# wathiede/pbrt

Hardware: AMD Instinct MI355X
Metric: Msamples/sec (rays/sec) at 1/2/4/8 GPUs; PSNR vs CPU reference (higher is better)
Workload: dtype f32

## Files before the change

pbrt_amd/csrc/kernel_walk.hpp:

```cpp
#pragma once
#include <cstdio>
#include <cstdlib>
#include <vector>

#include "device_types.h"
#include "kernel_math.hpp"

namespace pbrt_hip {
namespace {

constexpr uint32_t kDone = 0xffffffffu;

typedef __attribute__((address_space(3))) uint32_t lds_u32;
__device__ __forceinline__ uint32_t lds_addr(const uint32_t *p) { return (uint32_t)(uintptr_t)(const lds_u32 *)p; }
__device__ __forceinline__ void lds_store(uint32_t a, uint32_t v) { *(lds_u32 *)(uintptr_t)a = v; }
__device__ __forceinline__ uint32_t lds_load(uint32_t a) { return *(const lds_u32 *)(uintptr_t)a; }
constexpr uint32_t kRowBytes = 256u;
__device__ __forceinline__ uint32_t lane_here() { uint32_t l = threadIdx.x & 63u; asm volatile("" : "+v"(l)); return l; }
__device__ __forceinline__ uint32_t lds_row(uint32_t a, const uint32_t *stk) { return (a - lds_addr(stk - (threadIdx.x & 63u))) / kRowBytes; }

struct Trav {
  V3 o, d;
  float tmax;
  uint32_t cur;
  uint32_t sp;
  uint32_t any;
  HitRec h;
};

struct TravTuning {
  uint32_t min_walkers;
  uint32_t min_parked;
};

#ifndef PBRT_PRIO_FETCH
#define PBRT_PRIO_FETCH 3
#endif
#ifndef PBRT_PRIO_ARITH
#define PBRT_PRIO_ARITH 0
#endif
#ifndef PBRT_PRIO_SERVICE
#define PBRT_PRIO_SERVICE 1
#endif
__device__ __forceinline__ void wave_prio(int p) {
#ifndef PBRT_NO_PRIO
  switch (p) {
    case 0: __builtin_amdgcn_s_setprio(0); break;
    case 1: __builtin_amdgcn_s_setprio(1); break;
    case 2: __builtin_amdgcn_s_setprio(2); break;
    default: __builtin_amdgcn_s_setprio(3); break;
  }
#endif
}

__device__ __forceinline__ bool box_test(float lx, float ly, float lz, float hx, float hy, float hz, V3 o, V3 inv,
                                         bool negx, bool negy, bool negz, float tfar, float &tn) {
  const float nx = ((negx ? hx : lx) - o.x) * inv.x, fx = ((negx ? lx : hx) - o.x) * inv.x;
  const float ny = ((negy ? hy : ly) - o.y) * inv.y, fy = ((negy ? ly : hy) - o.y) * inv.y;
  const float nz = ((negz ? hz : lz) - o.z) * inv.z, fz = ((negz ? lz : hz) - o.z) * inv.z;
  tn = fmaxf(fmaxf(nx, ny), fmaxf(nz, kRayTMin));
  const float tf = fminf(fminf(fx, fy), fminf(fz, tfar));
  return tn <= tf * kBoxPad;
}

template <bool EXACT, uint32_t OVFR>
__device__ __forceinline__ uint32_t trav_pop(Trav &T, uint32_t *stk, float *stkt, uint32_t *ovf, unsigned long long &cn) {
  if (EXACT) {
    while (T.sp != 0u) {
      T.sp--;
      const uint32_t ref = stk[T.sp * 64u];
      const float tn = stkt[T.sp * 64u];
      cn++;
      if (tn <= fminf(T.h.t, T.tmax) * kBoxPad) return ref;
    }
    return kDone;
  }
  T.sp -= kRowBytes;
  if (OVFR == 0u) return lds_load(T.sp);
  const uint32_t e = lds_row(T.sp, stk);
  return e < OVFR - 1u ? lds_load(T.sp) : ovf[(e - (OVFR - 1u)) * 64u + lane_here()];
}
template <uint32_t OVFR>
__device__ __forceinline__ void trav_push(Trav &T, uint32_t *stk, uint32_t *ovf, uint32_t ref) {
  if (OVFR == 0u) {
    lds_store(T.sp, ref);
  } else {
    const uint32_t e = lds_row(T.sp, stk);
    if (e < OVFR - 1u) lds_store(T.sp, ref);
    else ovf[(e - (OVFR - 1u)) * 64u + lane_here()] = ref;
  }
  T.sp += kRowBytes;
}

__device__ __forceinline__ void trav_enter(Trav &T, uint32_t ref) { T.cur = ref; }
__device__ __forceinline__ bool trav_parked(const Trav &T) { return T.cur != kDone && (T.cur & kLeafRef) != 0u; }
__device__ __forceinline__ uint32_t trav_leaf_cnt(const Trav &T) { return trav_parked(T) ? (T.cur >> 24) & 0x7fu : 0u; }

#include "experiments.inc"
template <bool EXACT>
__device__ __forceinline__ void trav_begin(const DevScene &S, Trav &T, uint32_t *stk, V3 o, V3 d, float tmax, bool any,
                                           unsigned long long &cn) {
  T.o = o;
  T.d = d;
  T.tmax = tmax;
  T.sp = 0;
  if (!EXACT) {
    lds_store(lds_addr(stk), kDone);
    T.sp = lds_addr(stk) + kRowBytes;
  }
  T.any = any ? 1u : 0u;
  T.h.t = kInf;
  T.h.prim = kNoPrim;
  T.h.slot = kNoPrim;
  T.h.b1 = 0.f;
  T.h.b2 = 0.f;
  T.cur = kDone;
  if (S.n_nodes) {
    if (EXACT) cn++;
    if (!EXACT && o.x >= S.root_lo[0] && o.x <= S.root_hi[0] && o.y >= S.root_lo[1] && o.y <= S.root_hi[1] && o.z >= S.root_lo[2] &&
        o.z <= S.root_hi[2]) {
      trav_enter(T, !(S.root_ref & kLeafRef) ? 0u : S.root_ref);
      return;
    }
    const V3 inv = {1.0f / d.x, 1.0f / d.y, 1.0f / d.z};
    float tn;
    if (box_test(S.root_lo[0], S.root_lo[1], S.root_lo[2], S.root_hi[0], S.root_hi[1], S.root_hi[2], o, inv,
                 inv.x < 0.f, inv.y < 0.f, inv.z < 0.f, tmax, tn))
      trav_enter(T, (!EXACT && !(S.root_ref & kLeafRef)) ? 0u : S.root_ref);
  }
}

__device__ __forceinline__ V3 walk_inv(const V3 d, const V3 inv1, const float inv_parallel) {
  return V3{d.x == 0.f ? copysignf(inv_parallel, inv1.x) : inv1.x, d.y == 0.f ? copysignf(inv_parallel, inv1.y) : inv1.y,
            d.z == 0.f ? copysignf(inv_parallel, inv1.z) : inv1.z};
}

template <bool SCALAR_FMA>
__device__ __forceinline__ void quad_step(const uint4 W0, const uint4 W1, const uint4 W2, const V3 o, const V3 inv, const bool negx,
                                          const bool negy, const bool negz, const float tfar, float (&key)[4], bool (&hit)[4]) {
  const float gx = (o.x - __uint_as_float(W0.x)) * inv.x, gy = (o.y - __uint_as_float(W0.y)) * inv.y;
  const float gz = (o.z - __uint_as_float(W0.z)) * inv.z;
  constexpr float kMargin = 0x1.8p-22f;
  const float gxn = __builtin_fmaf(fabsf(gx), kMargin, gx), gxf = __builtin_fmaf(-fabsf(gx), kMargin, gx);
  const float gyn = __builtin_fmaf(fabsf(gy), kMargin, gy), gyf = __builtin_fmaf(-fabsf(gy), kMargin, gy);
  const float gzn = __builtin_fmaf(fabsf(gz), kMargin, gz), gzf = __builtin_fmaf(-fabsf(gz), kMargin, gz);
  const float cix = __uint_as_float(W0.w) * inv.x, ciy = __uint_as_float(W2.z) * inv.y, ciz = __uint_as_float(W2.w) * inv.z;
  const uint32_t bnx = negx ? W1.w : W1.x, bfx = negx ? W1.x : W1.w;
  const uint32_t bny = negy ? W2.x : W1.y, bfy = negy ? W1.y : W2.x;
  const uint32_t bnz = negz ? W2.y : W1.z, bfz = negz ? W1.z : W2.y;
  const f32x2 gxx = {gxn, gxf}, gyy = {gyn, gyf}, gzz = {gzn, gzf}, cxx = {cix, cix}, cyy = {ciy, ciy}, czz = {ciz, ciz};
#pragma unroll
  for (int k = 0; k < 4; k++) {
    const float qxn = (float)((bnx >> (8 * k)) & 0xffu), qxf = (float)((bfx >> (8 * k)) & 0xffu);
    const float qyn = (float)((bny >> (8 * k)) & 0xffu), qyf = (float)((bfy >> (8 * k)) & 0xffu);
    const float qzn = (float)((bnz >> (8 * k)) & 0xffu), qzf = (float)((bfz >> (8 * k)) & 0xffu);
    f32x2 tx, ty, tz;
    if (SCALAR_FMA) {
      tx = f32x2{__builtin_fmaf(qxn, cix, -gxn), __builtin_fmaf(qxf, cix, -gxf)};
      ty = f32x2{__builtin_fmaf(qyn, ciy, -gyn), __builtin_fmaf(qyf, ciy, -gyf)};
      tz = f32x2{__builtin_fmaf(qzn, ciz, -gzn), __builtin_fmaf(qzf, ciz, -gzf)};
    } else {
      tx = __builtin_elementwise_fma(f32x2{qxn, qxf}, cxx, -gxx);
      ty = __builtin_elementwise_fma(f32x2{qyn, qyf}, cyy, -gyy);
      tz = __builtin_elementwise_fma(f32x2{qzn, qzf}, czz, -gzz);
    }
    const float tn = fmaxf(fmaxf(tx.x, ty.x), fmaxf(tz.x, kRayTMin));
    const float tf = fminf(fminf(tx.y, ty.y), fminf(tz.y, tfar));
    hit[k] = tn <= tf * kBoxPad;
    key[k] = tn;
  }
}

template <bool EXACT, bool COUNT, uint32_t OVFR, int STEPS = PBRT_STEPS_PER_CHECK, bool SPH = false>
__device__ __forceinline__ void trav_run(const DevScene &S, Trav &T, uint32_t *stk, float *stkt, uint32_t *ovf,
                                         const bool alive, const TravTuning tune, unsigned long long &cn,
                                         unsigned long long &ct) {
  const V3 o = T.o, d = T.d;
  const V3 inv1 = {1.0f / d.x, 1.0f / d.y, 1.0f / d.z};
  const bool negx = inv1.x < 0.f, negy = inv1.y < 0.f, negz = inv1.z < 0.f;
  const uint32_t negbits = (negx ? 1u : 0u) | (negy ? 2u : 0u) | (negz ? 4u : 0u);
#ifdef PBRT_INV_INF
  const V3 inv = inv1;
#else
  const V3 inv = EXACT ? inv1 : walk_inv(d, inv1, S.inv_parallel);
#endif
  const char *nodes = reinterpret_cast<const char *>(S.nodes);
  const char *quads = reinterpret_cast<const char *>(S.quads);
  const char *tris = reinterpret_cast<const char *>(S.tris);
  for (;;) {
    const bool walking = T.cur != kDone;
    const unsigned long long mwalk = __ballot(walking);
    if (mwalk == 0ull) break;
    if ((uint32_t)__popcll(mwalk) * 64u < tune.min_walkers * (uint32_t)__popcll(__ballot(alive)) && __ballot(!walking && alive) != 0ull) break;

    if (EXACT && walking && !trav_parked(T)) {
      const uint32_t off = T.cur * 64u;
      const uint4 q0 = *reinterpret_cast<const uint4 *>(nodes + off);
      const uint4 q1 = *reinterpret_cast<const uint4 *>(nodes + off + 16u);
      const uint4 q2 = *reinterpret_cast<const uint4 *>(nodes + off + 32u);
      const uint4 q3 = *reinterpret_cast<const uint4 *>(nodes + off + 48u);
      const float tfar = fminf(T.h.t, T.tmax);
      const f32x2 lx = {__uint_as_float(q0.x), __uint_as_float(q1.z)}, hx = {__uint_as_float(q0.w), __uint_as_float(q2.y)};
      const f32x2 ly = {__uint_as_float(q0.y), __uint_as_float(q1.w)}, hy = {__uint_as_float(q1.x), __uint_as_float(q2.z)};
      const f32x2 lz = {__uint_as_float(q0.z), __uint_as_float(q2.x)}, hz = {__uint_as_float(q1.y), __uint_as_float(q2.w)};
      const f32x2 nx = ((negx ? hx : lx) - o.x) * inv.x, fx = ((negx ? lx : hx) - o.x) * inv.x;
      const f32x2 ny = ((negy ? hy : ly) - o.y) * inv.y, fy = ((negy ? ly : hy) - o.y) * inv.y;
      const f32x2 nz = ((negz ? hz : lz) - o.z) * inv.z, fz = ((negz ? lz : hz) - o.z) * inv.z;
      const float tn0 = fmaxf(fmaxf(nx.x, ny.x), fmaxf(nz.x, kRayTMin));
      const float tn1 = fmaxf(fmaxf(nx.y, ny.y), fmaxf(nz.y, kRayTMin));
      const float tf0 = fminf(fminf(fx.x, fy.x), fminf(fz.x, tfar));
      const float tf1 = fminf(fminf(fx.y, fy.y), fminf(fz.y, tfar));
      const bool hit0 = tn0 <= tf0 * kBoxPad, hit1 = tn1 <= tf1 * kBoxPad;
      const bool far_first = ((negbits >> q3.z) & 1u) != 0u;
      const uint32_t ref_near = far_first ? q3.y : q3.x, ref_far = far_first ? q3.x : q3.y;
      const bool hit_near = (far_first && hit1) || (!far_first && hit0);
      const bool hit_far = (far_first && hit0) || (!far_first && hit1);
      if (EXACT) {
        cn++;
        stk[T.sp * 64u] = ref_far;
        stkt[T.sp * 64u] = hit_far ? (far_first ? tn0 : tn1) : __builtin_nanf("");
        T.sp++;
      }
      trav_enter(T, hit_near ? ref_near : trav_pop<EXACT, OVFR>(T, stk, stkt, ovf, cn));
    }

#pragma unroll
    for (int rep = 0; !EXACT && rep < STEPS; rep++) {
    EXP_PROBE_LANES(0, T.cur != kDone && !trav_parked(T));
    if (T.cur != kDone && !trav_parked(T)) {
      const uint32_t off = T.cur;
      wave_prio(PBRT_PRIO_FETCH);
      const uint4 W0 = EXP_NODE_LOAD(reinterpret_cast<const uint4 *>(quads + off));
      const uint4 W1 = EXP_NODE_LOAD(reinterpret_cast<const uint4 *>(quads + off + 16u));
      const uint4 W2 = EXP_NODE_LOAD(reinterpret_cast<const uint4 *>(quads + off + 32u));
      const uint4 W3 = EXP_NODE_LOAD(reinterpret_cast<const uint4 *>(quads + off + 48u));
      EXP_STEP_EXTRA_LOADS(quads, off, T);
      wave_prio(PBRT_PRIO_ARITH);
      if (COUNT) cn++;
      const float tfar = fminf(T.h.t, T.tmax);
      EXP_STEP_EXTRA_VALU(W0, tfar, T);
      float key[4];
      bool hit[4];
      quad_step<OVFR == 0u>(W0, W1, W2, o, inv, negx, negy, negz, tfar, key, hit);
#ifdef PBRT_PRIO_SELECT
      wave_prio(PBRT_PRIO_SELECT);
#endif
#include "quad_nearest.inc"
      const bool any_hit = hit[0] || hit[1] || hit[2] || hit[3];
      const uint32_t nearest = n0 ? W3.x : (n1 ? W3.y : (n2 ? W3.z : W3.w));
      if (OVFR != 0u && __builtin_expect(__ballot(T.sp >= lds_addr(stk - (threadIdx.x & 63u)) + (OVFR - 4u) * kRowBytes) != 0ull, 0)) {
        if (hit[3] && !n3) trav_push<OVFR>(T, stk, ovf, W3.w);
        if (hit[2] && !n2) trav_push<OVFR>(T, stk, ovf, W3.z);
        if (hit[1] && !n1) trav_push<OVFR>(T, stk, ovf, W3.y);
        if (hit[0] && !n0) trav_push<OVFR>(T, stk, ovf, W3.x);
        trav_enter(T, any_hit ? nearest : trav_pop<false, OVFR>(T, stk, stkt, ovf, cn));
      } else {
        const uint32_t below = T.sp - kRowBytes, top = lds_load(below);
        const uint32_t next = any_hit ? nearest : top;
        lds_store(T.sp, W3.w); T.sp += (hit[3] && !n3) ? kRowBytes : 0u;
        lds_store(T.sp, W3.z); T.sp += (hit[2] && !n2) ? kRowBytes : 0u;
        lds_store(T.sp, W3.y); T.sp += (hit[1] && !n1) ? kRowBytes : 0u;
        lds_store(T.sp, W3.x); T.sp += (hit[0] && !n0) ? kRowBytes : 0u;
        T.sp = any_hit ? T.sp : below;
        trav_enter(T, next);
      }
    }
    }

    const bool parked = trav_parked(T);
    const unsigned long long mleaf = __ballot(parked);
    if (mleaf != 0ull &&
        ((uint32_t)__popcll(mleaf) >= tune.min_parked ||
         (uint32_t)__popcll(mleaf) * 2u >= (uint32_t)__popcll(__ballot(T.cur != kDone && !parked)))) {
      const uint32_t cnt = parked ? (T.cur >> 24) & 0x7fu : 0u, first = T.cur & 0xffffffu;
      bool stop = false;
      EXP_LEAF_PREFETCH_BEGIN(parked, quads, T);
      EXP_PROBE_FLUSH(cnt);
      for (uint32_t i = 0;; i++) {
        if (__ballot(cnt > i && !stop) == 0ull) break;
        EXP_PROBE_LANES(2, cnt > i && !stop);
        if (cnt > i && !stop) {
          const uint32_t slot = first + i;
          wave_prio(PBRT_PRIO_FETCH);
          const float4 a = EXP_TRI_LOAD(reinterpret_cast<const float4 *>(tris + slot * (16u * kTriStride)));
          const float4 b = EXP_TRI_LOAD(reinterpret_cast<const float4 *>(tris + slot * (16u * kTriStride) + 16u));
          const float4 c = EXP_TRI_LOAD(reinterpret_cast<const float4 *>(tris + slot * (16u * kTriStride) + 32u));
          wave_prio(PBRT_PRIO_ARITH);
          if (COUNT) ct++;
#include "tri_test.inc"
          float ht = tsnap, hu = u, hv = v;
          if (SPH && __float_as_uint(c.w) != 0u) {
            const float r = b.x;
            float ts = 0.f;
            valid = sphere_hit(make_float4(a.x, a.y, a.z, r), o, d, T.tmax, ts);
            const V3 lo = {a.x - r, a.y - r, a.z - r}, hi = {a.x + r, a.y + r, a.z + r};
            const float sx0 = (lo.x - o.x) * inv1.x, sx1 = (hi.x - o.x) * inv1.x, sy0 = (lo.y - o.y) * inv1.y, sy1 = (hi.y - o.y) * inv1.y;
            const float sz0 = (lo.z - o.z) * inv1.z, sz1 = (hi.z - o.z) * inv1.z;
            const float stn = fmaxf(fmaxf(fminf(fminf(sx0, sx1), sx0), fminf(fminf(sy0, sy1), sy0)), fmaxf(fminf(fminf(sz0, sz1), sz0), kRayTMin));
            const float stf = fminf(fminf(fmaxf(fmaxf(sx0, sx1), sx0), fmaxf(fmaxf(sy0, sy1), sy0)), fmaxf(fmaxf(sz0, sz1), sz0));
            ht = fmaxf(ts, stn);
            valid = valid && stn <= stf * kOwnPad && ht < T.tmax;
            hu = 0.f; hv = 0.f;
          }
          const uint32_t id = __float_as_uint(a.w);
          const bool occl = valid && T.any != 0u;
          const bool closer = valid && T.any == 0u && (ht < T.h.t || (ht == T.h.t && id < T.h.prim));
          T.any = occl ? 3u : T.any;
          stop = stop || occl;
          T.h.t = closer ? ht : T.h.t;
          T.h.prim = closer ? id : T.h.prim;
          T.h.slot = closer ? slot : T.h.slot;
          T.h.b1 = closer ? hu : T.h.b1;
          T.h.b2 = closer ? hv : T.h.b2;
        }
      }
      EXP_LEAF_PREFETCH_END();
      const bool far_pop = OVFR != 0u && !EXACT &&
                           __ballot(parked && !stop && T.sp >= lds_addr(stk - (threadIdx.x & 63u)) + OVFR * kRowBytes) != 0ull;
      if (parked) {
        if (stop) {
          T.cur = kDone;
          T.sp = 0u;
        } else if (OVFR != 0u && __builtin_expect(far_pop, 0)) {
          trav_enter(T, trav_pop<EXACT, OVFR>(T, stk, stkt, ovf, cn));
        } else {
          trav_enter(T, trav_pop<EXACT, 0u>(T, stk, stkt, ovf, cn));
        }
      }
    }
  }
}

}
}
```

Before: 468.4.

## Streamline wave votes, rotate walk loop, and peel first leaf triangle test

```diff
diff --git a/pbrt_amd/csrc/kernel_walk.hpp b/pbrt_amd/csrc/kernel_walk.hpp
--- a/pbrt_amd/csrc/kernel_walk.hpp
+++ b/pbrt_amd/csrc/kernel_walk.hpp
@@ -171,6 +171,14 @@
   }
 }
 
+__device__ __forceinline__ unsigned long long wave_vote(bool p) {
+#ifdef PBRT_WALK_MASKS_OLD
+  return __ballot(p);
+#else
+  return __builtin_amdgcn_ballot_w64(p);
+#endif
+}
+
 template <bool EXACT, bool COUNT, uint32_t OVFR, int STEPS = PBRT_STEPS_PER_CHECK, bool SPH = false>
 __device__ __forceinline__ void trav_run(const DevScene &S, Trav &T, uint32_t *stk, float *stkt, uint32_t *ovf,
                                          const bool alive, const TravTuning tune, unsigned long long &cn,
@@ -187,13 +195,34 @@
   const char *nodes = reinterpret_cast<const char *>(S.nodes);
   const char *quads = reinterpret_cast<const char *>(S.quads);
   const char *tris = reinterpret_cast<const char *>(S.tris);
+#ifndef PBRT_WALK_MASKS_OLD
+  const unsigned long long malive = wave_vote(alive);
+  const uint32_t walkers_x64 = tune.min_walkers * (uint32_t)__popcll(malive);
+#endif
+#ifndef PBRT_WALK_ROTATE_OLD
+  const auto go_on = [&]() -> bool {
+    const bool walking = T.cur != kDone;
+    const unsigned long long mwalk = wave_vote(walking);
+#ifdef PBRT_WALK_MASKS_OLD
+    return mwalk != 0ull && !((uint32_t)__popcll(mwalk) * 64u < tune.min_walkers * (uint32_t)__popcll(__ballot(alive)) && __ballot(!walking && alive) != 0ull);
+#else
+    return mwalk != 0ull && !((uint32_t)__popcll(mwalk) * 64u < walkers_x64 && (malive & ~mwalk) != 0ull);
+#endif
+  };
+  if (go_on()) do {
+#else
   for (;;) {
     const bool walking = T.cur != kDone;
-    const unsigned long long mwalk = __ballot(walking);
+    const unsigned long long mwalk = wave_vote(walking);
     if (mwalk == 0ull) break;
+#ifdef PBRT_WALK_MASKS_OLD
     if ((uint32_t)__popcll(mwalk) * 64u < tune.min_walkers * (uint32_t)__popcll(__ballot(alive)) && __ballot(!walking && alive) != 0ull) break;
-
-    if (EXACT && walking && !trav_parked(T)) {
+#else
+    if ((uint32_t)__popcll(mwalk) * 64u < walkers_x64 && (malive & ~mwalk) != 0ull) break;
+#endif
+#endif
+
+    if (EXACT && T.cur != kDone && !trav_parked(T)) {
       const uint32_t off = T.cur * 64u;
       const uint4 q0 = *reinterpret_cast<const uint4 *>(nodes + off);
       const uint4 q1 = *reinterpret_cast<const uint4 *>(nodes + off + 16u);
@@ -248,7 +277,7 @@
 #include "quad_nearest.inc"
       const bool any_hit = hit[0] || hit[1] || hit[2] || hit[3];
       const uint32_t nearest = n0 ? W3.x : (n1 ? W3.y : (n2 ? W3.z : W3.w));
-      if (OVFR != 0u && __builtin_expect(__ballot(T.sp >= lds_addr(stk - (threadIdx.x & 63u)) + (OVFR - 4u) * kRowBytes) != 0ull, 0)) {
+      if (OVFR != 0u && __builtin_expect(wave_vote(T.sp >= lds_addr(stk - (threadIdx.x & 63u)) + (OVFR - 4u) * kRowBytes) != 0ull, 0)) {
         if (hit[3] && !n3) trav_push<OVFR>(T, stk, ovf, W3.w);
         if (hit[2] && !n2) trav_push<OVFR>(T, stk, ovf, W3.z);
         if (hit[1] && !n1) trav_push<OVFR>(T, stk, ovf, W3.y);
@@ -268,55 +297,41 @@
     }
 
     const bool parked = trav_parked(T);
-    const unsigned long long mleaf = __ballot(parked);
+    const unsigned long long mleaf = wave_vote(parked);
     if (mleaf != 0ull &&
         ((uint32_t)__popcll(mleaf) >= tune.min_parked ||
-         (uint32_t)__popcll(mleaf) * 2u >= (uint32_t)__popcll(__ballot(T.cur != kDone && !parked)))) {
+         (uint32_t)__popcll(mleaf) * 2u >= (uint32_t)__popcll(wave_vote(T.cur != kDone && !parked)))) {
       const uint32_t cnt = parked ? (T.cur >> 24) & 0x7fu : 0u, first = T.cur & 0xffffffu;
       bool stop = false;
       EXP_LEAF_PREFETCH_BEGIN(parked, quads, T);
       EXP_PROBE_FLUSH(cnt);
-      for (uint32_t i = 0;; i++) {
-        if (__ballot(cnt > i && !stop) == 0ull) break;
+#ifndef PBRT_WALK_LEAF_LOOP_OLD
+      constexpr uint32_t kStraight = EXACT ? 0u : 1u;
+      if (!EXACT) {
+        constexpr uint32_t i = 0u;
+        EXP_PROBE_LANES(2, cnt != 0u);
+        if (cnt != 0u) {
+#include "leaf_test.inc"
+        }
+      }
+      if (EXACT || __builtin_expect(wave_vote(cnt > 1u) != 0ull, 0))
+#else
+      constexpr uint32_t kStraight = 0u;
+#endif
+      for (uint32_t i = kStraight;; i++) {
+        if (wave_vote(cnt > i && !stop) == 0ull) break;
         EXP_PROBE_LANES(2, cnt > i && !stop);
         if (cnt > i && !stop) {
-          const uint32_t slot = first + i;
-          wave_prio(PBRT_PRIO_FETCH);
-          const float4 a = EXP_TRI_LOAD(reinterpret_cast<const float4 *>(tris + slot * (16u * kTriStride)));
-          const float4 b = EXP_TRI_LOAD(reinterpret_cast<const float4 *>(tris + slot * (16u * kTriStride) + 16u));
-          const float4 c = EXP_TRI_LOAD(reinterpret_cast<const float4 *>(tris + slot * (16u * kTriStride) + 32u));
-          wave_prio(PBRT_PRIO_ARITH);
-          if (COUNT) ct++;
-#include "tri_test.inc"
-          float ht = tsnap, hu = u, hv = v;
-          if (SPH && __float_as_uint(c.w) != 0u) {
-            const float r = b.x;
-            float ts = 0.f;
-            valid = sphere_hit(make_float4(a.x, a.y, a.z, r), o, d, T.tmax, ts);
-            const V3 lo = {a.x - r, a.y - r, a.z - r}, hi = {a.x + r, a.y + r, a.z + r};
-            const float sx0 = (lo.x - o.x) * inv1.x, sx1 = (hi.x - o.x) * inv1.x, sy0 = (lo.y - o.y) * inv1.y, sy1 = (hi.y - o.y) * inv1.y;
-            const float sz0 = (lo.z - o.z) * inv1.z, sz1 = (hi.z - o.z) * inv1.z;
-            const float stn = fmaxf(fmaxf(fminf(fminf(sx0, sx1), sx0), fminf(fminf(sy0, sy1), sy0)), fmaxf(fminf(fminf(sz0, sz1), sz0), kRayTMin));
-            const float stf = fminf(fminf(fmaxf(fmaxf(sx0, sx1), sx0), fmaxf(fmaxf(sy0, sy1), sy0)), fmaxf(fmaxf(sz0, sz1), sz0));
-            ht = fmaxf(ts, stn);
-            valid = valid && stn <= stf * kOwnPad && ht < T.tmax;
-            hu = 0.f; hv = 0.f;
-          }
-          const uint32_t id = __float_as_uint(a.w);
-          const bool occl = valid && T.any != 0u;
-          const bool closer = valid && T.any == 0u && (ht < T.h.t || (ht == T.h.t && id < T.h.prim));
-          T.any = occl ? 3u : T.any;
-          stop = stop || occl;
-          T.h.t = closer ? ht : T.h.t;
-          T.h.prim = closer ? id : T.h.prim;
-          T.h.slot = closer ? slot : T.h.slot;
-          T.h.b1 = closer ? hu : T.h.b1;
-          T.h.b2 = closer ? hv : T.h.b2;
+#include "leaf_test.inc"
         }
       }
       EXP_LEAF_PREFETCH_END();
+#ifdef PBRT_WALK_MASKS_OLD
       const bool far_pop = OVFR != 0u && !EXACT &&
                            __ballot(parked && !stop && T.sp >= lds_addr(stk - (threadIdx.x & 63u)) + OVFR * kRowBytes) != 0ull;
+#else
+      const bool far_pop = OVFR != 0u && !EXACT && (wave_vote(T.sp >= lds_addr(stk - (threadIdx.x & 63u)) + OVFR * kRowBytes) & mleaf) != 0ull;
+#endif
       if (parked) {
         if (stop) {
           T.cur = kDone;
@@ -328,8 +343,12 @@
         }
       }
     }
-  }
-}
-
-}
-}
+#ifndef PBRT_WALK_ROTATE_OLD
+  } while (go_on());
+#else
+  }
+#endif
+}
+
+}
+}
```

Measured after the change: 488.8, median of 6. 1.04x the previous value.
